# allenai/aspire

Hardware: AMD Instinct MI355X
Metric: query x candidate OT alignments/sec (higher is better)
Workload: dtype f32; 1 GPU; otAspire compsci: 1 query x 1000 candidates per step (per GPU), 8 sents x 768d, Sinkhorn OT (blur 0.05, scaling 0.9, one eps schedule per pair) + stable top-100 rank; every step its own query and its own pool, 80 distinct pools (1877 MiB > 256 MiB L3) walked by consecutive calls; sents=8, dim=768, topk=100, parallelism=candidate-pool shards x1, streams=3

## Files before the change

aspire_amd/csrc/fused.hip:

```cpp
#include <math.h>

#include <mutex>

#include "common.h"
#include "score_device.h"
#include "score_types.h"
#include "fused_solve.h"
#include "tuning.h"

namespace aspire {
namespace {

#ifdef ASPIRE_PHASE_CLOCK
static __device__ long long* g_fdbg = nullptr;
#define F_STAMP(k)                                                                                                   \
    do {                                                                                                             \
        if (g_fdbg && lane == 0 && (k) < 8) g_fdbg[(size_t)(blockIdx.x * 4 + wave) * 8 + (k)] = (long long)__builtin_amdgcn_s_memrealtime(); \
    } while (0)
#else
#define F_STAMP(k) \
    do {           \
    } while (0)
#endif

// ... 351 lines not shown
        for (int k = 0; k < 2; ++k) nscr[(8 + k) * kNormLd + lane] = nx[k].x + nx[k].y;
        __builtin_amdgcn_fence(__ATOMIC_RELEASE, "wavefront");
        __builtin_amdgcn_wave_barrier();
        __builtin_amdgcn_fence(__ATOMIC_ACQUIRE, "wavefront");
        auto table_sum = [&](int value, int lane0) {
            const float4* src = reinterpret_cast<const float4*>(nscr + value * kNormLd + lane0);
            float t = 0.f;
#pragma unroll
            for (int m = 0; m < 4; ++m) {
                const float4 u = src[m];
                t += (u.x + u.y) + (u.z + u.w);
            }
            return t;
        };
        float xx[2], yy[2];
#pragma unroll
        for (int y = 0; y < 2; ++y) yy[y] = table_sum(2 * lj + y, p * 16);
#pragma unroll
        for (int x = 0; x < 2; ++x) xx[x] = table_sum(8 + ((2 * li + x) & 1), ((2 * li + x) >> 1) * 16);
        float diam2 = dsq.x + dsq.y;
        diam2 += lane_xor<1>(diam2); diam2 += lane_xor<2>(diam2); diam2 += lane_xor<4>(diam2); diam2 += lane_xor<8>(diam2);

        float cost[2][2], neg[2][2];
        bool redo[2][2];
#pragma unroll
        for (int x = 0; x < 2; ++x)
#pragma unroll
            for (int y = 0; y < 2; ++y) {
                const int i = 2 * li + x, j = row0 + 2 * lj + y;
                const float sq = fmaf(-2.f, accg[x][y], xx[x]) + yy[y];
                const float ns = xx[x] + yy[y];
                redo[x][y] = i < q_len && j < c_len && sq < 1e-4f * ns * ns;
                cost[x][y] = sqrtf(fmaxf(sq, 1e-8f));
                neg[x][y] = -sqrtf(fmaxf(sq, 0.f));
            }
        {
#pragma unroll
            for (int x = 0; x < 2; ++x)
#pragma unroll
                for (int y = 0; y < 2; ++y) {
                    unsigned long long wm = __ballot(redo[x][y]);
                    while (wm != 0) {
                        int owner[4];
                        float part[4];
#pragma unroll
                        for (int e = 0; e < 4; ++e) {
                            owner[e] = wm != 0 ? (int)__builtin_ctzll(wm) : -1;
                            wm = wm != 0 ? wm & (wm - 1) : 0;
                        }
                        float4 u[4][3], v[4][3];
#pragma unroll
                        for (int e = 0; e < 4; ++e) {
                            const int o = owner[e] >= 0 ? owner[e] : owner[0];
                            const int ol = o & 15, i = 2 * (ol >> 2) + x;
                            const int j = (CHUNK ? __builtin_amdgcn_readlane(row0, o) : 0) + 2 * (ol & 3) + y;
                            const int cs_e = __builtin_amdgcn_readlane(c_start, o);
                            const float* qrow = qdoc + (size_t)i * kD + 4 * lane;
                            const float* crow = a.c.rows + ((size_t)cs_e + j) * kD + 4 * lane;
// ... 40 lines not shown
            }
            const float diam = own_diam ? fmaxf(sqrtf(diam2), kMinDiameter) : a.diameter[q_idx * a.n_groups + c_idx / a.diam_group];
            solve_begin<CHUNK>(pend, a, cost, neg, rv, cv, diam, cw, cwide, row0 == 0);
            pend.out = (my_c_real && row0 == 0) ? (mapped ? c_idx : q_idx * a.c.n + c_idx) : (int64_t)-1;
            if (q_len > 8 || c_len > 8 * cur.gsz) pend.valid |= 16u;
            slice = (pend.max_steps + kStages - 1) / kStages;
            have_pend = true;
            F_STAMP(2 + 2 * n_done);
            ++n_done;
        } else if constexpr (L2MAX) {
            float m = kNegBig;
#pragma unroll
            for (int x = 0; x < 2; ++x)
#pragma unroll
                for (int y = 0; y < 2; ++y) m = fmaxf(m, (2 * li + x < q_len && row0 + 2 * lj + y < c_len) ? neg[x][y] : kNegBig);
            m = xg_max<CHUNK>(max_li(max_lj(m)), cw, cwide);
            if (q_len > 8 || c_len > 8 * cur.gsz) m = __builtin_nanf("");
            if (my_c_real && lp == 0 && row0 == 0) a.scores[mapped ? c_idx : q_idx * a.c.n + c_idx] = m;
        } else if (my_c_real && lp == 0) {
            a.scores[mapped ? c_idx : q_idx * a.c.n + c_idx] = diam2;
        }
    }
    F_STAMP(6);
    if constexpr (SOLVE)
        if (have_pend && !a.skip_tail) solve_finish<CHUNK>(pend, a);
    F_STAMP(7);
}

}

bool fused_self_ok(int64_t jobs, const aspire_ot_params* prm) {
    return jobs <= 64 && prm->scaling >= 0.25 && tuning().fused_nosolve != 1 && !tuning().fused_valu && !tuning().fused_noself;
}

bool fused_inbox_ok(const aspire_repset* q, const float* diameter) {
    return q->n == 1 && diameter == nullptr && tuning().fused_nosolve != 1 && !tuning().fused_valu && !tuning().fused_noself;
}

bool fused_path_ok(const aspire_repset* q, const aspire_repset* c) {
    const int mq = q->max_len, mc = c->max_len;
    return q->ext == 0 && c->ext == 0 && mq > 0 && mc > 0 && mq <= 8 && mc <= 8;
}

int launch_pair_fused_l2max(const ScoreArgs& a, int64_t groups_bound, hipStream_t stream, bool self) {
    const int64_t waves = groups_bound < 256 * 8 ? groups_bound : 256 * 8;
    const dim3 grid((unsigned)((waves + 3) / 4));
    if (self)
        hipLaunchKernelGGL((pair_fused_kernel<true, false, true, true>), grid, dim3(256), 4 * kWaveLds * sizeof(float), stream, a,
                           (const float*)nullptr);
    else
        hipLaunchKernelGGL((pair_fused_kernel<true, false, false, true>), grid, dim3(256), 4 * kWaveLds * sizeof(float), stream, a,
                           (const float*)nullptr);
    ASPIRE_LAUNCH_OK();
    return ASPIRE_OK;
}

int launch_pair_fused(const ScoreArgs& a_in, int64_t groups_bound, const float* qbox, hipStream_t stream) {
    ScoreArgs a = a_in;
    a.skip_tail = tuning().fused_nosolve == 2;
    const int64_t cap = tuning().fused_waves > 0 ? tuning().fused_waves : 256 * 8;
    const int64_t waves = groups_bound < cap ? groups_bound : cap;
    const dim3 grid((unsigned)((waves + 3) / 4));
    const bool self = qbox == nullptr && a.pairing == kPairMapped;
    const bool inbox1 = qbox == nullptr && a.pairing == ASPIRE_PAIR_CROSS;
    if ((self || inbox1) && (tuning().fused_nosolve == 1 || tuning().fused_valu)) return ASPIRE_ERR_INVALID_ARG;
    const size_t lds = 4 * (kWaveLds + (self || inbox1 ? 2 * kD : 0)) * sizeof(float);
    if (tuning().fused_nosolve == 1) hipLaunchKernelGGL((pair_fused_kernel<true, false>), grid, dim3(256), lds, stream, a, qbox);
    else if (tuning().fused_valu) hipLaunchKernelGGL((pair_fused_kernel<false, true>), grid, dim3(256), lds, stream, a, qbox);
    else if (self) {
        static std::once_flag raised;
        static hipError_t raise_rc = hipSuccess;
        std::call_once(raised, [] {
            raise_rc = hipFuncSetAttribute(reinterpret_cast<const void*>(pair_fused_kernel<true, true, true>),
                                           hipFuncAttributeMaxDynamicSharedMemorySize, 80 * 1024);
        });
        ASPIRE_HIP_OK(raise_rc);
        hipLaunchKernelGGL((pair_fused_kernel<true, true, true>), grid, dim3(256), lds, stream, a, qbox);
    }
    else if (inbox1) {
        static std::once_flag raised1;
        static hipError_t raise1_rc = hipSuccess;
        std::call_once(raised1, [] {
            raise1_rc = hipFuncSetAttribute(reinterpret_cast<const void*>(pair_fused_kernel<true, true, false, false, true>),
                                            hipFuncAttributeMaxDynamicSharedMemorySize, 80 * 1024);
        });
// ... 41 lines not shown
```

aspire_amd/csrc/fused_solve.h:

```cpp
#pragma once
#include <math.h>

#include "common.h"
#include "score_device.h"
#include "score_types.h"

namespace aspire {
namespace {

constexpr int kCh = 16;
constexpr int kStages = kD / (4 * kCh);
constexpr int kRowStride = 4 * kCh + 4;
constexpr int kRows = 8 + 8 * 4;
constexpr int kNormLd = 68;
constexpr int kNormOfs = 256;
constexpr int kWaveLds = kRows * kRowStride;
static_assert(kNormOfs + 16 * kNormLd <= kWaveLds, "norm table must fit the idle stage buffer");

typedef float mfma4_t __attribute__((ext_vector_type(4)));

__device__ __forceinline__ float vmin1(float a, float b) {
    float r;
    asm("v_min_f32 %0, %1, %2" : "=v"(r) : "v"(a), "v"(b));
    return r;
// ... 66 lines not shown
        }
    }
    return v;
}

typedef float f2_t __attribute__((ext_vector_type(2)));

struct Solve {
    f2_t mc[2];
    f2_t neg[2];
    f2_t wa, wb;
    f2_t f, g;
    float diam;
    float r2, h;
    int n_mid;
    int k, max_steps;
    int n_mid_lo;
    unsigned valid;
    int w;
    bool wide, first;
    int64_t out;
};

template <bool XG = false>
__device__ __forceinline__ void solve_begin(Solve& s, const ScoreArgs& a, const float (&cost)[2][2], const float (&neg)[2][2],
                                            const bool (&rv)[2], const bool (&cv)[2], float diam, int w = 1, bool wide = false,
                                            bool first = true) {
    s.w = w;
    s.wide = wide;
    s.first = first;
    s.diam = diam;
    const float temp = (float)a.temp;
    {
        float qm[2], cm[2];
#pragma unroll
        for (int x = 0; x < 2; ++x)
            qm[x] = xg_max<XG>(max_lj(fmaxf((rv[x] && cv[0]) ? neg[x][0] : kNegBig, (rv[x] && cv[1]) ? neg[x][1] : kNegBig)), w, wide) / temp;
#pragma unroll
        for (int y = 0; y < 2; ++y)
            cm[y] = max_li(fmaxf((rv[0] && cv[y]) ? neg[0][y] : kNegBig, (rv[1] && cv[y]) ? neg[1][y] : kNegBig)) / temp;
        const float mq = max_li(fmaxf(rv[0] ? qm[0] : kNegBig, rv[1] ? qm[1] : kNegBig));
        const float mc = xg_max<XG>(max_lj(fmaxf(cv[0] ? cm[0] : kNegBig, cv[1] ? cm[1] : kNegBig)), w, wide);
        const float sq = (rv[0] ? fast_exp(qm[0] - mq) : 0.f) + (rv[1] ? fast_exp(qm[1] - mq) : 0.f);
        const float sc = (cv[0] ? fast_exp(cm[0] - mc) : 0.f) + (cv[1] ? fast_exp(cm[1] - mc) : 0.f);
        const float lsq = fast_log(sum_li(sq)), lsc = fast_log(xg_sum<XG>(sum_lj(sc), w, wide));
#pragma unroll
        for (int t = 0; t < 2; ++t) {
            s.wa[t] = rv[t] ? fast_exp(qm[t] - mq - lsq) : 0.f;
            s.wb[t] = cv[t] ? fast_exp(cm[t] - mc - lsc) : 0.f;
        }
    }
    s.valid = (rv[0] ? 1u : 0u) | (rv[1] ? 2u : 0u) | (cv[0] ? 4u : 0u) | (cv[1] ? 8u : 0u);
    float ldf;
    s.n_mid = schedule_mid_steps(a, diam, ldf);
    int ms = s.n_mid, ml = s.n_mid;
    ms = max(ms, __shfl_xor(ms, 16));
    ms = max(ms, __shfl_xor(ms, 32));
    ml = min(ml, __shfl_xor(ml, 16));
    ml = min(ml, __shfl_xor(ml, 32));
    s.max_steps = __builtin_amdgcn_readfirstlane(ms) + 3;
    s.n_mid_lo = __builtin_amdgcn_readfirstlane(ml);
    s.k = 0;
    const float r2_first = kLog2e * rcp_refined(diam), h_first = 0.5f * kLn2 * diam;
    s.r2 = r2_first;
    s.h = h_first;
#pragma unroll
    for (int x = 0; x < 2; ++x) {
        s.mc[x] = f2_t{(rv[x] && cv[0]) ? cost[x][0] : 0.f, (rv[x] && cv[1]) ? cost[x][1] : 0.f};
        s.neg[x] = f2_t{(rv[x] && cv[0]) ? neg[x][0] : 0.f, (rv[x] && cv[1]) ? neg[x][1] : 0.f};
    }
    float rs[2] = {0.f, 0.f}, cs[2] = {0.f, 0.f};
#pragma unroll
    for (int x = 0; x < 2; ++x)
#pragma unroll
        for (int y = 0; y < 2; ++y) {
            const float k0 = __builtin_amdgcn_exp2f(-s.mc[x][y] * r2_first);
            rs[x] = fmaf(s.wb[y], k0, rs[x]);
            cs[y] = fmaf(s.wa[x], k0, cs[y]);
        }
#pragma unroll
    for (int t = 0; t < 2; ++t) {
        s.f[t] = -2.f * h_first * __builtin_amdgcn_logf(xg_sum<XG>(sum_lj(rs[t]), w, wide));
        s.g[t] = -2.f * h_first * __builtin_amdgcn_logf(sum_li(cs[t]));
    }
}

template <int W>
__device__ __forceinline__ float xg_sum_w(float v, bool wide) {
    if constexpr (W == 2) {
        const float s = swap_add<16>(v, v);
        v = wide ? s : v;
    } else if constexpr (W == 4) {
        float z = wide ? v : 0.f;
        z = swap_add<16>(z, z);
        z = swap_add<32>(z, z);
        v = wide ? z : v;
    }
    return v;
}
template <int W = 1>
__device__ __forceinline__ void solve_step(Solve& s, float r2, float h) {
    const f2_t fr = s.f * r2, gr = s.g * r2;
    const f2_t a0 = __builtin_elementwise_fma(s.mc[0], f2_t{-r2, -r2}, f2_t{fr.x, fr.x} + gr);
    const f2_t a1 = __builtin_elementwise_fma(s.mc[1], f2_t{-r2, -r2}, f2_t{fr.y, fr.y} + gr);
    const f2_t k0 = {__builtin_amdgcn_exp2f(a0.x), __builtin_amdgcn_exp2f(a0.y)};
    const f2_t k1 = {__builtin_amdgcn_exp2f(a1.x), __builtin_amdgcn_exp2f(a1.y)};
    const f2_t t0 = k0 * s.wb, t1 = k1 * s.wb;
// ... 132 lines not shown
            f[t] = mine ? 0.5f * (f[t] + ft[t]) : f[t];
            g[t] = mine ? 0.5f * (g[t] + gt[t]) : g[t];
        }
        if (k >= 1) eps *= scal;
    }
    softmins(eb, f, g, ft, gt);
    return solve_output<XG>(s, a, f2_t{ft[0], ft[1]}, f2_t{gt[0], gt[1]});
}

template <bool XG = false>
__device__ __forceinline__ void solve_finish(Solve& s, const ScoreArgs& a) {
    solve_steps<XG>(s, a, -1);
    float score = solve_output<XG>(s, a, s.f, s.g);
    bool bad = !(fabsf(score) < 1e30f);
    if (a.want != ASPIRE_OT_PLAN_SIM && (a.want == ASPIRE_OT_SIMILARITY ? score : -score) > 1e-2f) bad = true;
    if (__any(bad && !(s.valid & 16u))) {
        const float again = solve_safe<XG>(s, a);
        if (bad) score = again;
    }
    if (s.valid & 16u) score = __builtin_nanf("");
    if (s.out >= 0 && (threadIdx.x & 15) == 0) a.scores[s.out] = score;
}

}
}
```

aspire_amd/csrc/lib.hip:

```cpp
#include <stdarg.h>
#include <stdio.h>

#include <stdlib.h>
#include <string.h>

#include <mutex>

#include "common.h"
#include "tuning.h"

namespace aspire {
namespace {
thread_local char g_err[512] = "";
Tuning g_tuning;
std::once_flag g_tuning_once;

bool apply_tuning(Tuning& t, const char* key, const char* v) {
    const bool unset = !v || !*v;
    if (!strcmp(key, "SINKHORN")) {
        const int f = unset ? 0 : !strcmp(v, "wave") ? 1 : !strcmp(v, "block") ? 3 : !strcmp(v, "block-norepair") ? 4 : !strcmp(v, "block16") ? 5 : !strcmp(v, "block-dense") ? 6 : !strcmp(v, "block-wide") ? 7 : -1;
        if (f < 0) return false;
        t.sinkhorn_form = f;
    } else if (!strcmp(key, "COST_PATH")) {
        const int f = unset ? 0 : !strcmp(v, "mfma") ? 1 : !strcmp(v, "valu") ? 2 : -1;
// ... 11 lines not shown
        if (f < 0) return false;
        t.gemm_form = f;
    } else if (!strcmp(key, "GEMM_TILE")) {
        const int f = unset ? 0 : atoi(v);
        if (f != 0 && f != 96 && f != 128 && f != 64 && f != 256) return false;
        t.gemm_tile96 = f == 96;
        t.gemm_tile = f;
    } else if (!strcmp(key, "GEMM_RING")) {
        int f = unset ? 0 : atoi(v);
        if (f == 2 || f == 3) f += 20;
        if (f != 0 && f != 22 && f != 23 && f != 12 && f != 13 && f != 14 && f != 113) return false;
        t.gemm_ring = f;
    } else if (!strcmp(key, "GEMM_LN")) {
        if (!unset && strcmp(v, "off") && strcmp(v, "on")) return false;
        t.gemm_ln = unset ? 0 : !strcmp(v, "off") ? 1 : 2;
    } else if (!strcmp(key, "GEMM_PROBE")) {
        t.gemm_probe = unset ? 0 : atoi(v);
    } else if (!strcmp(key, "FUSED_VALU")) {
        t.fused_valu = unset ? 0 : atoi(v);
    } else if (!strcmp(key, "FUSED_NOSOLVE")) {
        t.fused_nosolve = unset ? 0 : atoi(v);
    } else if (!strcmp(key, "FUSED_NOSELF")) {
        t.fused_noself = unset ? 0 : atoi(v);
    } else if (!strcmp(key, "FUSED_WAVES")) {
        t.fused_waves = unset ? 0 : atoi(v);
    } else if (!strcmp(key, "FUSED_SPLIT")) {
        t.fused_split = unset ? 0 : atoi(v);
    } else if (!strcmp(key, "SPLIT_PRIO")) {
        t.split_prio = unset ? 0 : atoi(v);
    } else if (!strcmp(key, "GRAM_TILE")) {
        const int f = unset ? 0 : atoi(v);
        if (f != 0 && f != 128128 && f != 128256 && f != 256128 && f != 256256) return false;
        t.gram_tile = f;
    } else if (!strcmp(key, "GRAM_PP")) {
        t.gram_pp = unset ? 0 : atoi(v);
    } else if (!strcmp(key, "GRAM_RING")) {
        const int f = unset ? 0 : atoi(v);
        if (f != 0 && f != 3 && f != 4) return false;
        t.gram_ring = f;
    } else if (!strcmp(key, "OT_FORM")) {
        const int f = unset ? 0 : !strcmp(v, "small") ? 1 : !strcmp(v, "tile") ? 2 : !strcmp(v, "fused") ? 3 : !strcmp(v, "chunk") ? 4 : !strcmp(v, "one") ? 5 : -1;
        if (f < 0) return false;
        t.ot_form = f;
    } else {
        return false;
    }
// ... 1 lines not shown
}

bool render_tuning(const Tuning& t, const char* key, char* buf, size_t len) {
    const char* v = nullptr;
    char num[32] = "";
    auto number = [&](int n) {
        if (n != 0) snprintf(num, sizeof(num), "%d", n);
        return (const char*)num;
    };
    if (!strcmp(key, "SINKHORN")) {
        static const char* names[] = {"", "wave", "", "block", "block-norepair", "block16", "block-dense", "block-wide"};
        v = names[t.sinkhorn_form];
    } else if (!strcmp(key, "COST_PATH")) v = t.cost_path == 1 ? "mfma" : t.cost_path == 2 ? "valu" : "";
    else if (!strcmp(key, "COST1_BLOCKS")) v = number(t.cost1_blocks);
    else if (!strcmp(key, "ATTN")) v = t.attn_gemm ? "gemm" : t.attn_f32 ? "f32" : t.attn_form == 1 ? "f16x2" : t.attn_form == 2 ? "p64" : "";
    else if (!strcmp(key, "GEMM")) v = t.gemm_form == 1 ? "f32" : t.gemm_form == 2 ? "bf16x3" : t.gemm_form == 3 ? "planes" : "";
    else if (!strcmp(key, "GEMM_TILE")) v = number(t.gemm_tile);
    else if (!strcmp(key, "GEMM_RING")) v = number(t.gemm_ring);
    else if (!strcmp(key, "GEMM_LN")) v = t.gemm_ln == 1 ? "off" : t.gemm_ln == 2 ? "on" : "";
    else if (!strcmp(key, "GEMM_PROBE")) v = number(t.gemm_probe);
    else if (!strcmp(key, "FUSED_VALU")) v = number(t.fused_valu);
    else if (!strcmp(key, "FUSED_NOSOLVE")) v = number(t.fused_nosolve);
    else if (!strcmp(key, "FUSED_NOSELF")) v = number(t.fused_noself);
    else if (!strcmp(key, "FUSED_WAVES")) v = number(t.fused_waves);
    else if (!strcmp(key, "FUSED_SPLIT")) v = number(t.fused_split);
    else if (!strcmp(key, "SPLIT_PRIO")) v = number(t.split_prio);
    else if (!strcmp(key, "GRAM_TILE")) v = number(t.gram_tile);
    else if (!strcmp(key, "GRAM_RING")) v = number(t.gram_ring);
    else if (!strcmp(key, "GRAM_PP")) v = number(t.gram_pp);
    else if (!strcmp(key, "OT_FORM")) v = t.ot_form == 1 ? "small" : t.ot_form == 2 ? "tile" : t.ot_form == 3 ? "fused" : t.ot_form == 4 ? "chunk" : t.ot_form == 5 ? "one" : "";
    if (!v || strlen(v) + 1 > len) return false;
    strcpy(buf, v);
    return true;
}

void tuning_from_env() {
    static const char* keys[] = {"SINKHORN", "COST_PATH", "COST1_BLOCKS", "ATTN", "GEMM_TILE", "GEMM_RING", "GEMM_LN", "GEMM_PROBE", "GEMM", "OT_FORM", "FUSED_VALU", "FUSED_NOSOLVE", "FUSED_WAVES", "FUSED_SPLIT", "SPLIT_PRIO", "FUSED_NOSELF", "GRAM_TILE", "GRAM_RING", "GRAM_PP"};
    for (const char* k : keys) {
        char name[64];
        snprintf(name, sizeof(name), "ASPIRE_HIP_%s", k);
        if (const char* v = getenv(name)) apply_tuning(g_tuning, k, v);
    }
}
}

const Tuning& tuning() {
    std::call_once(g_tuning_once, tuning_from_env);
    return g_tuning;
}
bool tuning_set(const char* key, const char* value) {
    std::call_once(g_tuning_once, tuning_from_env);
    return apply_tuning(g_tuning, key, value);
}
bool tuning_get(const char* key, char* buf, size_t len) {
    std::call_once(g_tuning_once, tuning_from_env);
    return render_tuning(g_tuning, key, buf, len);
}

void set_error(const char* fmt, ...) {
    va_list ap;
// ... 99 lines not shown
```

aspire_amd/csrc/score.hip:

```cpp
#include <math.h>
#include <stdlib.h>
#include <string.h>

#include <type_traits>

#include "common.h"
#include "tuning.h"
#include "score_types.h"
#include "score_device.h"
#include "topk_device.h"
#include "batch_host.h"

namespace aspire {
namespace {

constexpr int64_t kStreamMinGroups1 = 640, kStreamMinGroupsBatch = 512;

int check_repsets(const aspire_repset* q, const aspire_repset* c, int64_t D, int pairing) {
    ASPIRE_REQUIRE(q && c, ASPIRE_ERR_INVALID_ARG, "null repset");
    ASPIRE_REQUIRE(D == kD, ASPIRE_ERR_UNSUPPORTED, "encoding dim %lld unsupported (kernels are built for 768)",
                   (long long)D);
    ASPIRE_REQUIRE(pairing == ASPIRE_PAIR_CROSS || pairing == ASPIRE_PAIR_PAIRED, ASPIRE_ERR_INVALID_ARG,
                   "bad pairing %d", pairing);
    ASPIRE_REQUIRE(q->n >= 0 && c->n >= 0, ASPIRE_ERR_INVALID_ARG, "negative document count");
// ... 229 lines not shown
    ws.cost = (float*)base;
    ws.neg = ws.cost + n_slots * PairWs<T>::kEntries;
    ws.diam2 = ws.neg + n_slots * PairWs<T>::kEntries;
    return ws;
}
}

namespace aspire {
namespace {

constexpr int64_t kChunkMinCands = 256;
bool chunk_size_ok(int64_t C) {
    const int form_t = tuning().ot_form;
    return form_t == 4 || (form_t == 0 && C >= kChunkMinCands);
}
constexpr int64_t kOneMinPairs = 1, kOneMaxPairs = 8192;
bool one_wave_form_ok(int64_t pairs, bool plain_call, bool small_grid) {
    const int form_t = tuning().ot_form;
    return plain_call && small_grid && pairs >= kOneMinPairs && pairs <= kOneMaxPairs &&
           (form_t == 5 || (form_t == 0 && tuning().sinkhorn_form == 0 && tuning().cost_path == 0 && tuning().cost1_blocks == 0));
}

struct BatchLayout {
    size_t slots, qbox, cand_job, grp_job, grp_off, grp_rec, gate, topk, total;
};
BatchLayout batch_layout(int64_t J, int64_t C, int max_rows, int64_t max_job, int64_t k) {
    BatchLayout L{};
    size_t o = 0;
    L.slots = o; o = align16(o + slot_bytes(max_rows) * (size_t)C);
    L.qbox = o; o = align16(o + (size_t)J * 2 * kD * sizeof(float));
    L.cand_job = o; o = align16(o + (size_t)C * sizeof(int32_t));
    L.grp_job = o; o = align16(o + (size_t)(C / 4 + J + 1) * sizeof(int32_t));
    L.grp_off = o; o = align16(o + (size_t)(J + 1 > 64 ? J + 1 : 64) * sizeof(int32_t));
    const size_t n_rec = max_rows > 16 ? 2 * (size_t)chunk_items_bound(J, C, max_job) + 1
                         : max_rows > 8 ? (size_t)chunk_items_bound(J, C, max_job) + 1 : (size_t)(C / 4 + J + 1);
    L.grp_rec = o; o = align16(o + n_rec * 16 * sizeof(int32_t));
    L.gate = o; o = align16(o + 16);
    L.topk = o; o = align16(o + aspire_topk_workspace_bytes(J, max_job, k));
    L.total = o;
    return L;
}
BatchLayout l2_batch_layout(int64_t J, int64_t C, int64_t max_job, int64_t k) {
    BatchLayout L{};
    size_t o = 0;
    L.cand_job = o; o = align16(o + (size_t)C * sizeof(int32_t));
    L.grp_job = o; o = align16(o + (size_t)(C / 4 + J + 1) * sizeof(int32_t));
    L.grp_off = o; o = align16(o + (size_t)(J + 1 > 64 ? J + 1 : 64) * sizeof(int32_t));
    L.grp_rec = o; o = align16(o + (2 * (size_t)chunk_items_bound(J, C, max_job) + 1) * 16 * sizeof(int32_t));
    L.qbox = o; o = align16(o + (size_t)J * 2 * kD * sizeof(float));
    L.gate = o; o = align16(o + 16);
    L.topk = o; o = align16(o + aspire_topk_workspace_bytes(J, max_job, k));
    L.total = o;
    return L;
}
BatchTables batch_tables(void* workspace, const BatchLayout& L) {
    char* w = (char*)workspace;
    return BatchTables{(float*)(w + L.slots), (float*)(w + L.qbox), (int32_t*)(w + L.cand_job), (int32_t*)(w + L.grp_job),
                       (int32_t*)(w + L.grp_off), (int32_t*)(w + L.grp_rec), (int32_t*)(w + L.gate), w + L.topk};
}
void fill_mapped_args(ScoreArgs& a, const BatchTables& t, const int32_t* job_off, int64_t J, int64_t C, int64_t max_job) {
    a.cand0 = 0;
    a.cand1 = C;
    a.qmap = t.cand_job;
    a.job_off = job_off;
    a.grp_off = t.grp_off;
    a.grp_job = t.grp_job;
    a.grp_rec = t.grp_rec;
    a.job0 = 0;
    a.job1 = (int32_t)J;
    a.max_job_groups = (int32_t)((max_job + 3) / 4);
}

int launch_fused_form(const ScoreArgs& a, int64_t groups, bool own_box, bool whole_call, const float* qbox, const aspire_ot_params* prm,
                      hipStream_t s) {
#ifdef ASPIRE_EXPERIMENT_SPLIT
    if (own_box && whole_call && split_path_ok(groups, prm) && a.c.n < ((int64_t)1 << 31) - 8) return launch_pair_split(a, s);
#endif
    return launch_pair_fused(a, groups, own_box ? nullptr : qbox, s);
}
}
}

namespace {

int ot_run_tiles(ScoreArgs a, const aspire_repset* q, const aspire_repset* c, const aspire_ot_params* prm, void* workspace,
                 size_t workspace_bytes, hipStream_t stream, bool cost_only) {
    const int pairing = a.pairing;
    const float* diameter = a.diameter;
    const bool extra = a.out_qdistr || a.out_cdistr || a.out_pairsims || a.out_plan;
    const int max_rows = max_rows_of(q, c);
    const size_t per_cand = per_cand_bytes(q, c, pairing);
    const bool planes_ot = !extra && gram_planes_wanted_ot(q, c, pairing, diameter != nullptr) && tuning().ot_form == 0;
    const bool stream16 = !planes_ot && q->n == 1 && c->n >= 4096 && tile16_path_ok(q, c, pairing) && tuning().cost_path != 1 &&
                          tuning().ot_form != 1;
    const int form_t = tuning().ot_form;
    const bool chunk1 = pairing == ASPIRE_PAIR_CROSS && q->n == 1 && q->ext == 0 && c->ext == 0 && q->max_len <= 8 && c->max_len > 8 &&
                        c->max_len <= 8 * kMaxT && c->n >= kChunkMinCands && c->n < ((int64_t)1 << 30) && !extra && !cost_only && !diameter &&
                        chunk_size_ok(c->n) && prm->scaling >= 0.25 && !tuning().fused_nosolve && !tuning().fused_valu &&
                        tuning().cost_path == 0 && workspace &&
                        (size_t)(chunk_items_bound(1, c->n, c->n) + 2) * 64 + 256 + qbox_bytes(q) + 64 <= workspace_bytes;
    const bool gram = (gram_path_wanted(q, c, pairing) || planes_ot) && !stream16 && !chunk1;
// ... 193 lines not shown
    const bool rec16 = max_rows > 16 && max_rows_all <= 8 * kMaxT && chunk_size_ok(C) && stages == kStageAll && tuning().cost_path != 2;
    if (rec16) {
        if (int rc = launch_rec_prep(a, t, job_off, J, max_job, s0)) return rc;
        const int rc_run = dispatch_T(max_rows, [&](auto tc) -> int {
            constexpr int T = decltype(tc)::value;
            if constexpr (T >= 3) {
                const PairWs<T> ws = pair_ws_at<T>(t.slots, C);
                if (int rc = launch_pair_tile16_rec(a, T, ws.cost, ws.neg, ws.diam2, 2 * chunk_items_bound(J, C, max_job), t.qbox, s0)) return rc;
                return launch_sinkhorn_stage(a, T, ws.cost, ws.neg, ws.diam2, C, max_rows, false, 3, s0);
            }
            return (int)ASPIRE_ERR_UNSUPPORTED;
        });
        if (rc_run) return rc_run;
        return rank.rank(scores);
    }
    const bool self = fused && fused_self_ok(J, prm);
    if ((stages & kStagePrep) && !self)
        if (int rc = launch_batch_tables(a, t, job_off, J, max_job, s0)) return rc;
    if (hybrid) {
        if (int rc = arm_long_pair_gate(a, t.gate, C, s0)) return rc;
        if (int rc = launch_pair_fused(a, groups_bound, t.qbox, s0)) return rc;
    }
    if (fused) {
        if (stages & (kStageCost | kStageSolve))
            if (int rc = launch_fused_form(a, groups_bound, self, stages == kStageAll, t.qbox, prm, s0)) return rc;
    } else {
        const int rc_run = dispatch_T(max_rows, [&](auto tc) -> int {
            constexpr int T = decltype(tc)::value;
            if constexpr (T == 1) {
                if (one_wave_form_ok(C, stages == kStageAll, !a.tile_form)) return launch_pair_one(a, C, s0);
            }
            const PairWs<T> ws = pair_ws_at<T>(t.slots, C);
            if (stages & kStageCost)
                if (int rc = launch_cost_stage(a, T, q, c, ws.cost, ws.neg, ws.diam2, C, 1, false, t.qbox, nullptr, true, s0)) return rc;
            if (stages & kStageSolve)
                if (int rc = launch_sinkhorn_stage(a, T, ws.cost, ws.neg, ws.diam2, C, max_rows, false, a.tile_form ? 3 : 0, s0)) return rc;
            return (int)ASPIRE_OK;
        });
        if (rc_run) return rc_run;
        if (max_rows_all > max_rows && (stages & kStageSolve))
            if (int rc = launch_pair_generic(a, 0, max_rows, q->max_len, c->max_len, s0)) return rc;
    }
    return rank.rank(scores);
}
}

// ... 101 lines not shown
```

aspire_amd/csrc/score_types.h:

```cpp
#pragma once
#include <type_traits>

#include "common.h"

namespace aspire {

struct RepSet {
    const float* rows;
    const int32_t* start;
    const int32_t* len;
    int64_t n;
    int32_t ext;
};

struct ScoreArgs {
    RepSet q, c;
    int pairing;
    int cdist_mode;
    int q_per_block;
    int64_t cand0, cand1;
    double blur, scaling, temp;
    double log_blur, log_scaling;
    float log2_blur, log2_scaling;
    const aspire_rep_planes* q_planes;
    const aspire_rep_planes* c_planes;
    const float* c_box;
    const float* diameter;
    int64_t diam_group;
    int64_t n_groups;
    int want;
    int agg;
    float* scores;
    float* out_qdistr;
    float* out_cdistr;
    float* out_pairsims;
    float* out_plan;
    const int32_t* qmap;
    const int32_t* job_off;
    const int32_t* grp_off;
    const int32_t* grp_job;
    const int32_t* grp_rec;
    int32_t job0, job1;
    int32_t max_job_groups;
    int32_t tile_form;
    int32_t cost_from_neg;
    int32_t skip_tail;
    int32_t chunk_regions, chunk_region_cap;
    int32_t center;
    const int32_t* gate;
    int32_t gate_limit;
    long long* dbg;
};

constexpr int kWaves = 3;
constexpr int kBlock = 64 * kWaves;
constexpr int kMaxT = 4;

constexpr int kPairMapped = 2;
constexpr float kMinDiameter = 1e-6f;

__device__ __forceinline__ bool gate_few_long(const ScoreArgs& a) { return a.gate != nullptr && *a.gate <= a.gate_limit; }

struct PairIdx {
    int64_t q_idx, c_idx, p;
};
__device__ __forceinline__ PairIdx pair_of_slot(const ScoreArgs& a, int64_t slot) {
    PairIdx r;
    if (a.pairing == ASPIRE_PAIR_CROSS) {
        const uint32_t ncand = (uint32_t)(a.cand1 - a.cand0);
// ... 31 lines not shown
    if (max_rows <= 8) return f(std::integral_constant<int, 1>{});
    if (max_rows <= 16) return f(std::integral_constant<int, 2>{});
    if (max_rows <= 24) return f(std::integral_constant<int, 3>{});
    if (max_rows <= 32) return f(std::integral_constant<int, 4>{});
    set_error("documents with more than %d sentence rows are not supported (got %d)", 8 * kMaxT, max_rows);
    return ASPIRE_ERR_UNSUPPORTED;
}

int launch_l2max_tiles(const ScoreArgs& a, int max_rows, int qchunks, hipStream_t stream);
int launch_doc_box(const RepSet& d, float* box, hipStream_t stream);
int launch_cost_stage(const ScoreArgs& a, int T, const aspire_repset* q, const aspire_repset* c, float* cost, float* neg, float* diam2,
                      int64_t n_slots, int qchunks, bool gram, float* qbox, float* cbox, bool first_chunk, hipStream_t stream);
int arm_long_pair_gate(ScoreArgs& a, int32_t* gate, int64_t C, hipStream_t stream);
int launch_group_diameter(const ScoreArgs& a, int64_t group, int64_t ngroups, int64_t blocks, float* diameter, hipStream_t stream);

int launch_sinkhorn_stage(const ScoreArgs& a, int T, float* cost, float* neg, float* diam2, int64_t n_slots, int max_rows, bool extra,
                          int form_hint, hipStream_t stream);
int launch_pair_one(const ScoreArgs& a, int64_t n_slots, hipStream_t stream);

struct BatchTables {
    float* slots;
    float* qbox;
    int32_t *cand_job, *grp_job, *grp_off, *grp_rec, *gate;
    void* topk;
};
int64_t chunk_items_bound(int64_t J, int64_t C, int64_t max_job);
int launch_batch_tables(const ScoreArgs& a, const BatchTables& t, const int32_t* job_off, int64_t J, int64_t max_job, hipStream_t stream);
int launch_chunk_prep(ScoreArgs& a, const BatchTables& t, const int32_t* job_off, int64_t J, int64_t max_job, hipStream_t stream);
int launch_rec_prep(const ScoreArgs& a, const BatchTables& t, const int32_t* job_off, int64_t J, int64_t max_job, hipStream_t stream);

bool gram_path_wanted(const aspire_repset* q, const aspire_repset* c, int pairing);
bool gram_planes_wanted_l2max(const aspire_repset* q, const aspire_repset* c, int pairing);
bool gram_planes_wanted_ot(const aspire_repset* q, const aspire_repset* c, int pairing, bool caller_diameters);
size_t gram_extra_bytes_per_cand(void);
int launch_pair_gram_ot(const ScoreArgs& a, int T, int mr_q, int mr_c, float* cost, float* neg, float* diam2, float* qbox,
                        float* cbox, hipStream_t stream);
int launch_pair_gram_l2max(const ScoreArgs& a, int mr_q, int mr_c, hipStream_t stream);

bool gram_planes_ok(const ScoreArgs& a);
struct GramGeometry {
    int mr_q, mr_c, dpt_q, dpt_c, n_qt, n_ct, E, ld;
    int bm, bn;
};
int launch_pair_gram_planes(const ScoreArgs& a, const GramGeometry& geo, bool l2max, float* cost, float* neg, hipStream_t stream);

int generic_max_rows(void);
int launch_pair_generic(const ScoreArgs& a, int mode, int skip_up_to, int rows_q, int rows_c, hipStream_t stream);

int launch_l2agg_backward(const RepSet& q, const RepSet& c, int agg, float temp, const float* grad_scores, float* grad_q, float* grad_c,
                          int rows_q, int rows_c, hipStream_t stream);

int launch_ot_backward(const RepSet& q, const RepSet& c, const aspire_ot_params* prm, const float* diameter, int64_t diam_group, int want,
                       const float* grad_scores, float* grad_q, float* grad_c, int rows_q, int rows_c, hipStream_t stream);

int launch_jointsm_backward(const RepSet& q, const RepSet& c, const float* grad_scores, float* grad_q, float* grad_c, int rows_q,
                            int rows_c, hipStream_t stream);

int launch_l2sup_scores(const RepSet& q, const RepSet& c, const int32_t* align, int weighted, float* scores, int rows_q, int rows_c,
                        hipStream_t stream);
int launch_l2sup_backward(const RepSet& q, const RepSet& c, const int32_t* align, int weighted, const float* grad_scores, float* grad_q,
                          float* grad_c, int rows_q, int rows_c, hipStream_t stream);

bool fused_self_ok(int64_t jobs, const aspire_ot_params* prm);
bool fused_inbox_ok(const aspire_repset* q, const float* diameter);
bool fused_path_ok(const aspire_repset* q, const aspire_repset* c);
int launch_pair_fused(const ScoreArgs& a, int64_t groups_bound, const float* qbox, hipStream_t stream);
#ifdef ASPIRE_EXPERIMENT_SPLIT
bool split_path_ok(int64_t groups_bound, const aspire_ot_params* prm);
int launch_pair_split(const ScoreArgs& a, hipStream_t stream);
#endif
int launch_pair_fused_chunk(const ScoreArgs& a, int64_t items_bound, const float* qbox, hipStream_t stream);
int launch_pair_fused_chunk_l2max(const ScoreArgs& a, int64_t items_bound, hipStream_t stream);
int launch_pair_fused_l2max(const ScoreArgs& a, int64_t groups_bound, hipStream_t stream, bool self = false);
bool tile16_path_ok(const aspire_repset* q, const aspire_repset* c, int pairing);
int launch_pair_tile16_l2max(const ScoreArgs& a, int64_t items_bound, hipStream_t stream);
int launch_pair_tile16(const ScoreArgs& a, float* cost, float* neg, float* diam2, int64_t items_bound, const float* qbox,
                       hipStream_t stream);
int launch_pair_tile16_rec(const ScoreArgs& a, int T, float* cost, float* neg, float* diam2, int64_t items_bound, const float* qbox,
                           hipStream_t stream);
int launch_pair_tile16_rec_l2max(const ScoreArgs& a, int64_t items_bound, hipStream_t stream);

}
```

aspire_amd/csrc/tuning.h:

```cpp
#pragma once

namespace aspire {

struct Tuning {
    int sinkhorn_form = 0;
    int cost_path = 0;
    int cost1_blocks = 0;
    int attn_f32 = 0;
    int attn_gemm = 0;
    int attn_form = 0;
    int gemm_form = 0;
    int gemm_tile96 = 0;
    int gemm_probe = 0;
    int gemm_ring = 0;
    int gemm_ln = 0;
    int gemm_tile = 0;
    int ot_form = 0;
    int fused_valu = 0;
    int fused_nosolve = 0;
    int fused_noself = 0;
    int gram_tile = 0;
    int gram_pp = 0;
    int gram_ring = 0;
    int fused_waves = 0;
    int fused_split = 0;
    int split_prio = 0;
};

const Tuning& tuning();
bool tuning_set(const char* key, const char* value);
bool tuning_get(const char* key, char* buf, unsigned long len);

}
```

Before: 165.0 million alignments/s.

## Add optional split finish kernel for fused Sinkhorn tail and cheaper cost sqrt

```diff
diff --git a/aspire_amd/csrc/fused.hip b/aspire_amd/csrc/fused.hip
--- a/aspire_amd/csrc/fused.hip
+++ b/aspire_amd/csrc/fused.hip
@@ -397,7 +397,8 @@
         diam2 += lane_xor<1>(diam2); diam2 += lane_xor<2>(diam2); diam2 += lane_xor<4>(diam2); diam2 += lane_xor<8>(diam2);
 
         float cost[2][2], neg[2][2];
-        bool redo[2][2];
+        bool redo[2][2], low[2][2];
+        float sqs[2][2];
 #pragma unroll
         for (int x = 0; x < 2; ++x)
 #pragma unroll
@@ -406,9 +407,18 @@
                 const float sq = fmaf(-2.f, accg[x][y], xx[x]) + yy[y];
                 const float ns = xx[x] + yy[y];
                 redo[x][y] = i < q_len && j < c_len && sq < 1e-4f * ns * ns;
-                cost[x][y] = sqrtf(fmaxf(sq, 1e-8f));
-                neg[x][y] = -sqrtf(fmaxf(sq, 0.f));
-            }
+                cost[x][y] = sqrtf(fmaxf(sq, 0.f));
+                neg[x][y] = -cost[x][y];
+                low[x][y] = !(sq >= 1e-8f);
+                sqs[x][y] = sq;
+            }
+        if (__any(low[0][0] || low[0][1] || low[1][0] || low[1][1])) {
+#pragma unroll
+            for (int x = 0; x < 2; ++x)
+#pragma unroll
+                for (int y = 0; y < 2; ++y)
+                    if (low[x][y]) cost[x][y] = sqrtf(fmaxf(sqs[x][y], 1e-8f));
+        }
         {
 #pragma unroll
             for (int x = 0; x < 2; ++x)
@@ -495,9 +505,23 @@
         }
     }
     F_STAMP(6);
-    if constexpr (SOLVE)
+    if constexpr (SOLVE) {
+        if constexpr (MFMA && !CHUNK && !QBOX) {
+            if (a.tail_rec != nullptr) {
+                tail_store(pend, a, have_pend, blockIdx.x * 4 + wave);
+                F_STAMP(7);
+                return;
+            }
+        }
         if (have_pend && !a.skip_tail) solve_finish<CHUNK>(pend, a);
+    }
     F_STAMP(7);
+}
+
+__global__ void __launch_bounds__(64) __attribute__((amdgpu_waves_per_eu(8, 8))) fused_finish_kernel(ScoreArgs a) {
+    Solve s;
+    if (!tail_load(s, a, blockIdx.x)) return;
+    solve_finish<false>(s, a);
 }
 
 }
@@ -528,12 +552,28 @@
     return ASPIRE_OK;
 }
 
+static int64_t fused_launch_waves(int64_t groups_bound) {
+    const int64_t cap = tuning().fused_waves > 0 ? tuning().fused_waves : 256 * 8;
+    const int64_t waves = groups_bound < cap ? groups_bound : cap;
+    return (waves + 3) / 4 * 4;
+}
+
+size_t fused_tail_bytes(int64_t groups_bound) { return (size_t)fused_launch_waves(groups_bound) * kTailRecFloats * sizeof(float); }
+
+bool fused_finish_ok(void) { return tuning().fused_finish && tuning().fused_nosolve == 0 && !tuning().fused_valu; }
+
+int launch_pair_fused_finish(const ScoreArgs& a, int64_t groups_bound, hipStream_t stream) {
+    if (a.tail_rec == nullptr) return ASPIRE_ERR_INVALID_ARG;
+    hipLaunchKernelGGL(fused_finish_kernel, dim3((unsigned)fused_launch_waves(groups_bound)), dim3(64), 0, stream, a);
+    ASPIRE_LAUNCH_OK();
+    return ASPIRE_OK;
+}
+
 int launch_pair_fused(const ScoreArgs& a_in, int64_t groups_bound, const float* qbox, hipStream_t stream) {
     ScoreArgs a = a_in;
     a.skip_tail = tuning().fused_nosolve == 2;
-    const int64_t cap = tuning().fused_waves > 0 ? tuning().fused_waves : 256 * 8;
-    const int64_t waves = groups_bound < cap ? groups_bound : cap;
-    const dim3 grid((unsigned)((waves + 3) / 4));
+    if (a.tail_rec != nullptr && (a.pairing != kPairMapped || a.gate != nullptr || !fused_finish_ok())) return ASPIRE_ERR_INVALID_ARG;
+    const dim3 grid((unsigned)(fused_launch_waves(groups_bound) / 4));
     const bool self = qbox == nullptr && a.pairing == kPairMapped;
     const bool inbox1 = qbox == nullptr && a.pairing == ASPIRE_PAIR_CROSS;
     if ((self || inbox1) && (tuning().fused_nosolve == 1 || tuning().fused_valu)) return ASPIRE_ERR_INVALID_ARG;
diff --git a/aspire_amd/csrc/fused_solve.h b/aspire_amd/csrc/fused_solve.h
--- a/aspire_amd/csrc/fused_solve.h
+++ b/aspire_amd/csrc/fused_solve.h
@@ -112,35 +112,8 @@
     int64_t out;
 };
 
-template <bool XG = false>
-__device__ __forceinline__ void solve_begin(Solve& s, const ScoreArgs& a, const float (&cost)[2][2], const float (&neg)[2][2],
-                                            const bool (&rv)[2], const bool (&cv)[2], float diam, int w = 1, bool wide = false,
-                                            bool first = true) {
-    s.w = w;
-    s.wide = wide;
-    s.first = first;
+__device__ __forceinline__ void solve_schedule(Solve& s, const ScoreArgs& a, float diam) {
     s.diam = diam;
-    const float temp = (float)a.temp;
-    {
-        float qm[2], cm[2];
-#pragma unroll
-        for (int x = 0; x < 2; ++x)
-            qm[x] = xg_max<XG>(max_lj(fmaxf((rv[x] && cv[0]) ? neg[x][0] : kNegBig, (rv[x] && cv[1]) ? neg[x][1] : kNegBig)), w, wide) / temp;
-#pragma unroll
-        for (int y = 0; y < 2; ++y)
-            cm[y] = max_li(fmaxf((rv[0] && cv[y]) ? neg[0][y] : kNegBig, (rv[1] && cv[y]) ? neg[1][y] : kNegBig)) / temp;
-        const float mq = max_li(fmaxf(rv[0] ? qm[0] : kNegBig, rv[1] ? qm[1] : kNegBig));
-        const float mc = xg_max<XG>(max_lj(fmaxf(cv[0] ? cm[0] : kNegBig, cv[1] ? cm[1] : kNegBig)), w, wide);
-        const float sq = (rv[0] ? fast_exp(qm[0] - mq) : 0.f) + (rv[1] ? fast_exp(qm[1] - mq) : 0.f);
-        const float sc = (cv[0] ? fast_exp(cm[0] - mc) : 0.f) + (cv[1] ? fast_exp(cm[1] - mc) : 0.f);
-        const float lsq = fast_log(sum_li(sq)), lsc = fast_log(xg_sum<XG>(sum_lj(sc), w, wide));
-#pragma unroll
-        for (int t = 0; t < 2; ++t) {
-            s.wa[t] = rv[t] ? fast_exp(qm[t] - mq - lsq) : 0.f;
-            s.wb[t] = cv[t] ? fast_exp(cm[t] - mc - lsc) : 0.f;
-        }
-    }
-    s.valid = (rv[0] ? 1u : 0u) | (rv[1] ? 2u : 0u) | (cv[0] ? 4u : 0u) | (cv[1] ? 8u : 0u);
     float ldf;
     s.n_mid = schedule_mid_steps(a, diam, ldf);
     int ms = s.n_mid, ml = s.n_mid;
@@ -151,14 +124,15 @@
     s.max_steps = __builtin_amdgcn_readfirstlane(ms) + 3;
     s.n_mid_lo = __builtin_amdgcn_readfirstlane(ml);
     s.k = 0;
-    const float r2_first = kLog2e * rcp_refined(diam), h_first = 0.5f * kLn2 * diam;
-    s.r2 = r2_first;
-    s.h = h_first;
-#pragma unroll
-    for (int x = 0; x < 2; ++x) {
-        s.mc[x] = f2_t{(rv[x] && cv[0]) ? cost[x][0] : 0.f, (rv[x] && cv[1]) ? cost[x][1] : 0.f};
-        s.neg[x] = f2_t{(rv[x] && cv[0]) ? neg[x][0] : 0.f, (rv[x] && cv[1]) ? neg[x][1] : 0.f};
-    }
+    s.r2 = kLog2e * rcp_refined(diam);
+    s.h = 0.5f * kLn2 * diam;
+}
+
+template <bool XG = false>
+__device__ __forceinline__ void solve_init(Solve& s) {
+    const float r2_first = s.r2, h_first = s.h;
+    const int w = s.w;
+    const bool wide = s.wide;
     float rs[2] = {0.f, 0.f}, cs[2] = {0.f, 0.f};
 #pragma unroll
     for (int x = 0; x < 2; ++x)
@@ -173,6 +147,43 @@
         s.f[t] = -2.f * h_first * __builtin_amdgcn_logf(xg_sum<XG>(sum_lj(rs[t]), w, wide));
         s.g[t] = -2.f * h_first * __builtin_amdgcn_logf(sum_li(cs[t]));
     }
+}
+
+template <bool XG = false>
+__device__ __forceinline__ void solve_begin(Solve& s, const ScoreArgs& a, const float (&cost)[2][2], const float (&neg)[2][2],
+                                            const bool (&rv)[2], const bool (&cv)[2], float diam, int w = 1, bool wide = false,
+                                            bool first = true) {
+    s.w = w;
+    s.wide = wide;
+    s.first = first;
+    const float temp = (float)a.temp;
+    {
+        float qm[2], cm[2];
+#pragma unroll
+        for (int x = 0; x < 2; ++x)
+            qm[x] = xg_max<XG>(max_lj(fmaxf((rv[x] && cv[0]) ? neg[x][0] : kNegBig, (rv[x] && cv[1]) ? neg[x][1] : kNegBig)), w, wide) / temp;
+#pragma unroll
+        for (int y = 0; y < 2; ++y)
+            cm[y] = max_li(fmaxf((rv[0] && cv[y]) ? neg[0][y] : kNegBig, (rv[1] && cv[y]) ? neg[1][y] : kNegBig)) / temp;
+        const float mq = max_li(fmaxf(rv[0] ? qm[0] : kNegBig, rv[1] ? qm[1] : kNegBig));
+        const float mc = xg_max<XG>(max_lj(fmaxf(cv[0] ? cm[0] : kNegBig, cv[1] ? cm[1] : kNegBig)), w, wide);
+        const float sq = (rv[0] ? fast_exp(qm[0] - mq) : 0.f) + (rv[1] ? fast_exp(qm[1] - mq) : 0.f);
+        const float sc = (cv[0] ? fast_exp(cm[0] - mc) : 0.f) + (cv[1] ? fast_exp(cm[1] - mc) : 0.f);
+        const float lsq = fast_log(sum_li(sq)), lsc = fast_log(xg_sum<XG>(sum_lj(sc), w, wide));
+#pragma unroll
+        for (int t = 0; t < 2; ++t) {
+            s.wa[t] = rv[t] ? fast_exp(qm[t] - mq - lsq) : 0.f;
+            s.wb[t] = cv[t] ? fast_exp(cm[t] - mc - lsc) : 0.f;
+        }
+    }
+    s.valid = (rv[0] ? 1u : 0u) | (rv[1] ? 2u : 0u) | (cv[0] ? 4u : 0u) | (cv[1] ? 8u : 0u);
+    solve_schedule(s, a, diam);
+#pragma unroll
+    for (int x = 0; x < 2; ++x) {
+        s.mc[x] = f2_t{(rv[x] && cv[0]) ? cost[x][0] : 0.f, (rv[x] && cv[1]) ? cost[x][1] : 0.f};
+        s.neg[x] = f2_t{(rv[x] && cv[0]) ? neg[x][0] : 0.f, (rv[x] && cv[1]) ? neg[x][1] : 0.f};
+    }
+    solve_init<XG>(s);
 }
 
 template <int W>
@@ -351,5 +362,67 @@
     if (s.out >= 0 && (threadIdx.x & 15) == 0) a.scores[s.out] = score;
 }
 
-}
-}
+constexpr int kTailRecFloats = 768;
+constexpr int kTailMarg = 256, kTailPair = 320, kTailHead = 336, kTailNeg = 512;
+
+__device__ __forceinline__ void tail_store(const Solve& s, const ScoreArgs& a, bool have, uint32_t slot) {
+    float* rec = a.tail_rec + (size_t)slot * kTailRecFloats;
+    const int lane = threadIdx.x & 63, p = lane >> 4, lp = lane & 15, li = lp >> 2, lj = lp & 3;
+    int4* head = reinterpret_cast<int4*>(rec + kTailHead);
+    if (!have) {
+        if (lane == 0) head[0] = make_int4(0, 0, 0, 0);
+        return;
+    }
+    unsigned long long b[5];
+#pragma unroll
+    for (int i = 0; i < 5; ++i) b[i] = __ballot(((s.valid >> i) & 1u) != 0);
+    if (lane == 0) {
+        head[0] = make_int4(1, 0, (int)(uint32_t)b[0], (int)(uint32_t)(b[0] >> 32));
+        head[1] = make_int4((int)(uint32_t)b[1], (int)(uint32_t)(b[1] >> 32), (int)(uint32_t)b[2], (int)(uint32_t)(b[2] >> 32));
+        head[2] = make_int4((int)(uint32_t)b[3], (int)(uint32_t)(b[3] >> 32), (int)(uint32_t)b[4], (int)(uint32_t)(b[4] >> 32));
+    }
+    *reinterpret_cast<float4*>(rec + 4 * lane) = make_float4(s.mc[0].x, s.mc[0].y, s.mc[1].x, s.mc[1].y);
+    if (a.want == ASPIRE_OT_PLAN_SIM)
+        *reinterpret_cast<float4*>(rec + kTailNeg + 4 * lane) = make_float4(s.neg[0].x, s.neg[0].y, s.neg[1].x, s.neg[1].y);
+    if (lj == 0) *reinterpret_cast<float2*>(rec + kTailMarg + 16 * p + 2 * li) = make_float2(s.wa.x, s.wa.y);
+    if (li == 0) *reinterpret_cast<float2*>(rec + kTailMarg + 16 * p + 8 + 2 * lj) = make_float2(s.wb.x, s.wb.y);
+    if (lp == 0)
+        *reinterpret_cast<int4*>(rec + kTailPair + 4 * p) =
+            make_int4(__float_as_int(s.diam), 0, (int)(uint32_t)(uint64_t)s.out, (int)(uint32_t)((uint64_t)s.out >> 32));
+}
+
+__device__ __forceinline__ bool tail_load(Solve& s, const ScoreArgs& a, uint32_t slot) {
+    const float* rec = a.tail_rec + (size_t)slot * kTailRecFloats;
+    const int lane = threadIdx.x & 63, p = lane >> 4, lp = lane & 15, li = lp >> 2, lj = lp & 3;
+    const int4* head = reinterpret_cast<const int4*>(rec + kTailHead);
+    const int4 h0 = head[0];
+    if (__builtin_amdgcn_readfirstlane(h0.x) == 0) return false;
+    const int4 h1 = head[1], h2 = head[2];
+    const float4 mc = *reinterpret_cast<const float4*>(rec + 4 * lane);
+    float4 ng = make_float4(0.f, 0.f, 0.f, 0.f);
+    if (a.want == ASPIRE_OT_PLAN_SIM) ng = *reinterpret_cast<const float4*>(rec + kTailNeg + 4 * lane);
+    const float2 wa = *reinterpret_cast<const float2*>(rec + kTailMarg + 16 * p + 2 * li);
+    const float2 wb = *reinterpret_cast<const float2*>(rec + kTailMarg + 16 * p + 8 + 2 * lj);
+    const int4 pr = *reinterpret_cast<const int4*>(rec + kTailPair + 4 * p);
+    const bool hi = lane >= 32;
+    const int bl[5] = {hi ? h0.w : h0.z, hi ? h1.y : h1.x, hi ? h1.w : h1.z, hi ? h2.y : h2.x, hi ? h2.w : h2.z};
+    s.valid = 0;
+#pragma unroll
+    for (int i = 0; i < 5; ++i) s.valid |= (((uint32_t)bl[i] >> (lane & 31)) & 1u) << i;
+    s.mc[0] = f2_t{mc.x, mc.y};
+    s.mc[1] = f2_t{mc.z, mc.w};
+    s.neg[0] = f2_t{ng.x, ng.y};
+    s.neg[1] = f2_t{ng.z, ng.w};
+    s.wa = f2_t{wa.x, wa.y};
+    s.wb = f2_t{wb.x, wb.y};
+    s.w = 1;
+    s.wide = false;
+    s.first = true;
+    s.out = (int64_t)(((uint64_t)(uint32_t)pr.w << 32) | (uint64_t)(uint32_t)pr.z);
+    solve_schedule(s, a, __int_as_float(pr.x));
+    solve_init<false>(s);
+    return true;
+}
+
+}
+}
diff --git a/aspire_amd/csrc/lib.hip b/aspire_amd/csrc/lib.hip
--- a/aspire_amd/csrc/lib.hip
+++ b/aspire_amd/csrc/lib.hip
@@ -57,6 +57,9 @@
         t.fused_nosolve = unset ? 0 : atoi(v);
     } else if (!strcmp(key, "FUSED_NOSELF")) {
         t.fused_noself = unset ? 0 : atoi(v);
+    } else if (!strcmp(key, "FUSED_FINISH")) {
+        if (!unset && strcmp(v, "off") && strcmp(v, "on")) return false;
+        t.fused_finish = !unset && !strcmp(v, "on");
     } else if (!strcmp(key, "FUSED_WAVES")) {
         t.fused_waves = unset ? 0 : atoi(v);
     } else if (!strcmp(key, "FUSED_SPLIT")) {
@@ -104,6 +107,7 @@
     else if (!strcmp(key, "FUSED_VALU")) v = number(t.fused_valu);
     else if (!strcmp(key, "FUSED_NOSOLVE")) v = number(t.fused_nosolve);
     else if (!strcmp(key, "FUSED_NOSELF")) v = number(t.fused_noself);
+    else if (!strcmp(key, "FUSED_FINISH")) v = t.fused_finish ? "on" : "";
     else if (!strcmp(key, "FUSED_WAVES")) v = number(t.fused_waves);
     else if (!strcmp(key, "FUSED_SPLIT")) v = number(t.fused_split);
     else if (!strcmp(key, "SPLIT_PRIO")) v = number(t.split_prio);
@@ -117,7 +121,7 @@
 }
 
 void tuning_from_env() {
-    static const char* keys[] = {"SINKHORN", "COST_PATH", "COST1_BLOCKS", "ATTN", "GEMM_TILE", "GEMM_RING", "GEMM_LN", "GEMM_PROBE", "GEMM", "OT_FORM", "FUSED_VALU", "FUSED_NOSOLVE", "FUSED_WAVES", "FUSED_SPLIT", "SPLIT_PRIO", "FUSED_NOSELF", "GRAM_TILE", "GRAM_RING", "GRAM_PP"};
+    static const char* keys[] = {"SINKHORN", "COST_PATH", "COST1_BLOCKS", "ATTN", "GEMM_TILE", "GEMM_RING", "GEMM_LN", "GEMM_PROBE", "GEMM", "OT_FORM", "FUSED_VALU", "FUSED_NOSOLVE", "FUSED_WAVES", "FUSED_SPLIT", "SPLIT_PRIO", "FUSED_NOSELF", "FUSED_FINISH", "GRAM_TILE", "GRAM_RING", "GRAM_PP"};
     for (const char* k : keys) {
         char name[64];
         snprintf(name, sizeof(name), "ASPIRE_HIP_%s", k);
diff --git a/aspire_amd/csrc/score.hip b/aspire_amd/csrc/score.hip
--- a/aspire_amd/csrc/score.hip
+++ b/aspire_amd/csrc/score.hip
@@ -275,7 +275,7 @@
 }
 
 struct BatchLayout {
-    size_t slots, qbox, cand_job, grp_job, grp_off, grp_rec, gate, topk, total;
+    size_t slots, qbox, cand_job, grp_job, grp_off, grp_rec, gate, tail, topk, total;
 };
 BatchLayout batch_layout(int64_t J, int64_t C, int max_rows, int64_t max_job, int64_t k) {
     BatchLayout L{};
@@ -289,6 +289,7 @@
                          : max_rows > 8 ? (size_t)chunk_items_bound(J, C, max_job) + 1 : (size_t)(C / 4 + J + 1);
     L.grp_rec = o; o = align16(o + n_rec * 16 * sizeof(int32_t));
     L.gate = o; o = align16(o + 16);
+    L.tail = o; o = align16(o + (max_rows <= 8 ? fused_tail_bytes(J * ((max_job + 3) / 4)) : 0));
     L.topk = o; o = align16(o + aspire_topk_workspace_bytes(J, max_job, k));
     L.total = o;
     return L;
@@ -309,7 +310,7 @@
 BatchTables batch_tables(void* workspace, const BatchLayout& L) {
     char* w = (char*)workspace;
     return BatchTables{(float*)(w + L.slots), (float*)(w + L.qbox), (int32_t*)(w + L.cand_job), (int32_t*)(w + L.grp_job),
-                       (int32_t*)(w + L.grp_off), (int32_t*)(w + L.grp_rec), (int32_t*)(w + L.gate), w + L.topk};
+                       (int32_t*)(w + L.grp_off), (int32_t*)(w + L.grp_rec), (int32_t*)(w + L.gate), (float*)(w + L.tail), w + L.topk};
 }
 void fill_mapped_args(ScoreArgs& a, const BatchTables& t, const int32_t* job_off, int64_t J, int64_t C, int64_t max_job) {
     a.cand0 = 0;
@@ -329,7 +330,8 @@
 #ifdef ASPIRE_EXPERIMENT_SPLIT
     if (own_box && whole_call && split_path_ok(groups, prm) && a.c.n < ((int64_t)1 << 31) - 8) return launch_pair_split(a, s);
 #endif
-    return launch_pair_fused(a, groups, own_box ? nullptr : qbox, s);
+    if (int rc = launch_pair_fused(a, groups, own_box ? nullptr : qbox, s)) return rc;
+    return a.tail_rec != nullptr ? launch_pair_fused_finish(a, groups, s) : (int)ASPIRE_OK;
 }
 }
 }
@@ -569,6 +571,7 @@
         if (int rc = launch_pair_fused(a, groups_bound, t.qbox, s0)) return rc;
     }
     if (fused) {
+        if ((stages & kStageCost) && (stages & kStageSolve) && fused_finish_ok()) a.tail_rec = t.tail;
         if (stages & (kStageCost | kStageSolve))
             if (int rc = launch_fused_form(a, groups_bound, self, stages == kStageAll, t.qbox, prm, s0)) return rc;
     } else {
diff --git a/aspire_amd/csrc/score_types.h b/aspire_amd/csrc/score_types.h
--- a/aspire_amd/csrc/score_types.h
+++ b/aspire_amd/csrc/score_types.h
@@ -45,6 +45,7 @@
     int32_t tile_form;
     int32_t cost_from_neg;
     int32_t skip_tail;
+    float* tail_rec;
     int32_t chunk_regions, chunk_region_cap;
     int32_t center;
     const int32_t* gate;
@@ -122,6 +123,7 @@
     float* slots;
     float* qbox;
     int32_t *cand_job, *grp_job, *grp_off, *grp_rec, *gate;
+    float* tail;
     void* topk;
 };
 int64_t chunk_items_bound(int64_t J, int64_t C, int64_t max_job);
@@ -165,6 +167,9 @@
 bool fused_inbox_ok(const aspire_repset* q, const float* diameter);
 bool fused_path_ok(const aspire_repset* q, const aspire_repset* c);
 int launch_pair_fused(const ScoreArgs& a, int64_t groups_bound, const float* qbox, hipStream_t stream);
+size_t fused_tail_bytes(int64_t groups_bound);
+bool fused_finish_ok(void);
+int launch_pair_fused_finish(const ScoreArgs& a, int64_t groups_bound, hipStream_t stream);
 #ifdef ASPIRE_EXPERIMENT_SPLIT
 bool split_path_ok(int64_t groups_bound, const aspire_ot_params* prm);
 int launch_pair_split(const ScoreArgs& a, hipStream_t stream);
diff --git a/aspire_amd/csrc/tuning.h b/aspire_amd/csrc/tuning.h
--- a/aspire_amd/csrc/tuning.h
+++ b/aspire_amd/csrc/tuning.h
@@ -19,6 +19,7 @@
     int fused_valu = 0;
     int fused_nosolve = 0;
     int fused_noself = 0;
+    int fused_finish = 0;
     int gram_tile = 0;
     int gram_pp = 0;
     int gram_ring = 0;
```

After: 160.3 million alignments/s. 2.9% lower.
